# zju3dv/ENeRF

Hardware: AMD Instinct MI355X
Metric: rendered frames/sec @512x640 3-src-view (higher is better)
Workload: dtype f32

## Files before the change

enerf_amd/csrc/render.hip:

```cpp
#include "nerf_layout.h"

#ifndef ENERF_RENDER_PREFETCH
#define ENERF_RENDER_PREFETCH 0
#endif

namespace enerf {

__host__ __device__ __forceinline__ int bx_image_floats(int F, int pieces = 3) { return F == 11 ? bx_layout().tiles * 256 * pieces : 0; }
long long nerf_packed_floats(int F) { return nerf_layout(F).total + bx_image_floats(F); }

__host__ __device__ __forceinline__ int slot_channel(int g, int r, int R, int F) {
    int c = g * R + r;
    return (r < R && c < F) ? c : -1;
}

__device__ __forceinline__ float bx_weight(const NerfRaw& w, int F, int e, int g, int j, int q) {
    const int R = (F + 3) / 4, CI = 88 + F + 4;
    const BxLayout B = bx_layout();
    const int half = q >> 2, r = q & 3;
    const int c = (r < R && g * R + r < F) ? g * R + r : -1;
    if (e < B.ga) return c >= 0 ? w.glob_w[(16 * e + j) * 3 * F + (1 + half) * F + c] : 0.f;
    if (e < B.fc) return (half == 0 && c >= 0) ? w.glob_w[(16 * (e - B.ga) + j) * 3 * F + c] : 0.f;
    if (e < B.lr0) return w.fc_w[j * 32 + 16 * half + 4 * g + r];
    if (e < B.c0p) {
// ... 21 lines not shown
    int i = blockIdx.x * blockDim.x + threadIdx.x;
    if (i >= L.total + bx_image_floats(F)) return;
    if (i >= L.total) {
        const int idx = i - L.total, n_plane = bx_layout().tiles * 256;
        const int piece = idx / n_plane, k = idx - piece * n_plane;
        const int e = k >> 8, lane = (k >> 2) & 63, wq = k & 3;
        unsigned word = 0;
        for (int h = 0; h < 2; ++h) {
            float rem = bx_weight(w, F, e, lane >> 4, lane & 15, 2 * wq + h);
            unsigned bits = 0;
            for (int pc = 0; pc <= piece; ++pc) { bits = bf16_bits_rne(rem); rem -= __uint_as_float(bits << 16); }
            word |= (bits & 0xffffu) << (16 * h);
        }
        out[i] = __uint_as_float(word);
        return;
    }
    const int R = L.R;
    const int CI = 88 + F + 4;
    float v = 0.f;
    auto mfma_lane = [&](int rel, int& e, int& g, int& row) { e = rel >> 6; g = (rel & 63) >> 4; row = rel & 15; };
    int e, g, row;
    if (i >= L.col2) {
        int k = i - L.col2;
        if (k < 64) v = w.col2_w[k]; else if (k == 64) v = w.col2_b[0];
    } else if (i >= L.c0v) {
        mfma_lane(i - L.c0v, e, g, row);
        int ks = e >> 2, vt = e & 3, unit = 16 * vt + row;
        if (ks < R) { int c = slot_channel(g, ks, R, F); if (c >= 0) v = w.col0_w[unit * CI + 88 + c]; }
        else if (ks == R) v = w.col0_w[unit * CI + 88 + F + g];
    } else if (i >= L.c0b) {
        int k = i - L.c0b; if (k < 64) v = w.col0_b[k];
    } else if (i >= L.c0p) {
        mfma_lane(i - L.c0p, e, g, row);
        int ks = e >> 2, vt = e & 3, unit = 16 * vt + row;
        if (ks < 16) v = w.col0_w[unit * CI + 16 * (ks >> 2) + 4 * g + (ks & 3)];
        else if (ks < 18) v = w.col0_w[unit * CI + 64 + 2 * g + (ks - 16)];
        else if (ks < 22) v = w.col0_w[unit * CI + 72 + 4 * g + (ks - 18)];
    } else if (i >= L.sigma) {
        int k = i - L.sigma;
        if (k < 64) v = w.sigma_w[k]; else if (k == 64) v = w.sigma_b[0];
    } else if (i >= L.lr0b) {
        int k = i - L.lr0b; if (k < 64) v = w.lr0_b[k];
    } else if (i >= L.lr0) {
        mfma_lane(i - L.lr0, e, g, row);
        int ks = e >> 2, vt = e & 3, unit = 16 * vt + row;
        if (ks < 2) v = w.lr0_w[unit * 24 + 2 * g + ks];
        else if (ks < 6) v = w.lr0_w[unit * 24 + 8 + 4 * g + (ks - 2)];
    } else if (i >= L.fcb) {
        int k = i - L.fcb; if (k < 16) v = w.fc_b[k];
    } else if (i >= L.fc) {
        mfma_lane(i - L.fc, e, g, row);
        if (e < 8) v = w.fc_w[row * 32 + 16 * (e >> 2) + 4 * g + (e & 3)];
    } else if (i >= L.aggw) {
        int k = i - L.aggw;
        if (k < 32) v = w.aggw_w[k]; else if (k == 32) v = w.aggw_b[0];
    } else if (i >= L.globb) {
        int k = i - L.globb; if (k < 32) v = w.glob_b[k];
    } else if (i >= L.glob) {
        mfma_lane(i - L.glob, e, g, row);
        int u = e & 1, pr = e >> 1, part = pr / R, r = pr - part * R;
        int c = slot_channel(g, r, R, F);
        if (part < 3 && c >= 0) v = w.glob_w[(16 * u + row) * 3 * F + part * F + c];
    } else if (i >= L.viewb) {
        int k = i - L.viewb;
        int t = k >> 4, rr = k & 15;
        int c = slot_channel(rr >> 2, 4 * t + (rr & 3), R, F);
        if (t < L.TR && c >= 0 && viewdir_agg) v = w.view_b[c];
    } else {
        mfma_lane(i - L.view, e, g, row);
        int c = slot_channel(row >> 2, 4 * e + (row & 3), R, F);
        if (e < L.TR && c >= 0 && viewdir_agg) v = w.view_w[c * 4 + g];
    }
    out[i] = v;
}
void launch_nerf_pack(const NerfRaw& raw, int F, int viewdir_agg, float* packed, hipStream_t st) {
    int total = (int)nerf_packed_floats(F);
    ENERF_LAUNCH_SIMPLE(k_nerf_pack, cdiv(total, 256), 256, 0, st, raw, F, viewdir_agg, packed);
}

constexpr int kCamStride = 16;

template <int R> struct Stage { static constexpr int kTex = 4 * R, kStride = 4 * R + 8; };

template <int R, int S, int WAVES, int WPE, bool PFK = false, bool LEANK = false, int BX = 0, bool RAW = false>
__global__ __launch_bounds__(64 * WAVES)
#ifndef ENERF_EMU
__attribute__((amdgpu_waves_per_eu(WPE, WPE)))
#endif
void k_render_rays(RenderArgs a) {
    static_assert(BX == 0 || R == 3, "the bf16 image exists for F = 11 only");
    static_assert(!RAW || (BX == 0 && !PFK), "raw samples come from the exact fp32 kernel, one sample at a time");
    constexpr bool BX3 = BX != 0;
    constexpr int NP = BX == 6 ? 3 : 2;
    constexpr int TR = (R + 3) / 4;
    constexpr int TEX = Stage<R>::kTex, SST = Stage<R>::kStride;
    const NerfLayout LF = nerf_layout(a.F);
    const NerfLayout L = nerf_layout(a.F, BX3);
    constexpr int BXP = 25 * 256;
    constexpr int BXF = BX3 ? BXP * NP : 0;
    ENERF_DYN_SMEM(float, smem);
    float* wl = smem;
    const float* bx = smem + L.total;
    auto bxplane = [&](int q) { return bx + q * BXP; };
    float* cam = smem + L.total + BXF;
    float* tcen = cam + a.B * S * kCamStride;
    float* stage_all = tcen + ((a.B * 4 + 15) & ~15);

    {
        constexpr int MAXW4 = (BX3 ? BXF : (R == 3 ? 10560 : 14528)) / 4;
        constexpr int NWI = (MAXW4 + 64 * WAVES - 1) / (64 * WAVES);
        float4 wq[NWI];
        const int n4 = (BX3 ? BXF : L.total) / 4;
        const float* src = a.packed + (BX3 ? LF.total : 0);
        float* dst = BX3 ? smem + L.total : wl;
#pragma unroll
        for (int it = 0; it < NWI; ++it) {
            const int i = (int)threadIdx.x + it * 64 * WAVES;
            wq[it] = *reinterpret_cast<const float4*>(src + (i < n4 ? i : n4 - 1) * 4);
        }
#pragma unroll
        for (int it = 0; it < NWI; ++it) {
            const int i = (int)threadIdx.x + it * 64 * WAVES;
            if (i < n4) *reinterpret_cast<float4*>(dst + i * 4) = wq[it];
        }
        if (BX3) {
            const int so[9] = {LF.view, LF.viewb, LF.globb, LF.aggw, LF.fcb, LF.lr0b, LF.sigma, LF.c0b, LF.col2};
            const int dd[9] = {L.view, L.viewb, L.globb, L.aggw, L.fcb, L.lr0b, L.sigma, L.c0b, L.col2};
            const int nn[9] = {L.TR * 64, L.TR * 16, 32, 33, 16, 64, 65, 64, 65};
            for (int q = 0; q < 9; ++q)
                for (int i = threadIdx.x; i < nn[q]; i += blockDim.x) wl[dd[q] + i] = a.packed[so[q] + i];
        }
    }
    for (int i = threadIdx.x; i < a.B * (S + 1); i += blockDim.x) {
        int b = i / (S + 1), s = i - b * (S + 1);
        const float* E = (s < S) ? a.src_exts + ((long long)b * S + s) * 16 : a.tar_ext + (long long)b * 16;
        double m[16], inv[16];
        for (int k = 0; k < 16; ++k) m[k] = (double)E[k];
        bool ok = inv4x4(m, inv);
        float c0 = ok ? (float)inv[3] : NAN, c1 = ok ? (float)inv[7] : NAN, c2 = ok ? (float)inv[11] : NAN;
        if (s < S) {
            float* c = cam + ((long long)b * S + s) * kCamStride;
            const float* K = a.src_ixts + ((long long)b * S + s) * 9;
            for (int r = 0; r < 3; ++r) {
                double kr[3];
                for (int q = 0; q < 3; ++q) kr[q] = (double)K[r * 3 + q] * (r < 2 ? (double)a.render_scale : 1.0);
                for (int q = 0; q < 4; ++q) {
                    const double v = kr[0] * m[q] + kr[1] * m[4 + q] + kr[2] * m[8 + q];
                    if (q < 3) c[r * 3 + q] = (float)v; else c[9 + r] = (float)v;
                }
            }
            c[12] = c0; c[13] = c1; c[14] = c2; c[15] = 0.f;
        } else {
            tcen[b * 4 + 0] = c0; tcen[b * 4 + 1] = c1; tcen[b * 4 + 2] = c2; tcen[b * 4 + 3] = 0.f;
        }
    }
    __syncthreads();

    const int lane = threadIdx.x & 63, g = lane >> 4, j = lane & 15;
    const int wave_in_block = threadIdx.x >> 6;
    const long long nrays = a.ray_index != nullptr ? (long long)a.ray_count[0] : (long long)a.B * a.N;
    const long long ntiles = cdivl(nrays, 16);
    const bool scatter = a.ray_index != nullptr && a.scatter_rgb != 0;
    const int Ns = a.n_samples;
    const float* wlane = wl + lane;
#define A_VIEW(e) wlane[L.view + (e) * 64]
#define A_GLOB(e) wlane[L.glob + (e) * 64]
#define A_FC(e) wlane[L.fc + (e) * 64]
#define A_LR0(e) wlane[L.lr0 + (e) * 64]
#define A_C0P(e) wlane[L.c0p + (e) * 64]
#define A_C0V(e) wlane[L.c0v + (e) * 64]
    float* stage = stage_all + wave_in_block * ((PFK ? 2 : 1) * S * 16 * SST);
    const int sv = g < S ? g : S - 1;
    float* my_rec = stage + (sv * 16 + j) * SST;
    const float* rd_rec = stage + j * SST + g * R;
    const float* rd_dir = stage + j * SST + TEX + g;

    const long long nbands = gridDim.x < 8 ? gridDim.x : 8;
    const long long xcd_ = blockIdx.x % nbands, nb8 = ((long long)gridDim.x + nbands - 1 - xcd_) / nbands, bi_ = blockIdx.x / nbands;
    const long long t_hi = ntiles * (xcd_ + 1) / nbands;
#ifndef ENERF_RENDER_BALANCE_R9
#define ENERF_RENDER_BALANCE_R9 1
#endif
    const long long t_lo = ntiles * xcd_ / nbands, per_round = nb8 * WAVES, full = (t_hi - t_lo) / per_round;
    const long long rem = (t_hi - t_lo) - full * per_round, rb = rem / nb8, rx = rem - rb * nb8;
    const long long my_rem = rb + (bi_ < rx ? 1 : 0), my_rem_lo = bi_ * rb + (bi_ < rx ? bi_ : rx);
    constexpr bool kBal = R == 3 || ENERF_RENDER_BALANCE_R9;
    const long long n_it = kBal ? full + (wave_in_block < my_rem ? 1 : 0)
                                : full + (full * per_round + bi_ * WAVES + wave_in_block < t_hi - t_lo ? 1 : 0);
    for (long long it = 0; it < n_it; ++it) {
        const long long tile = (it < full || !kBal) ? t_lo + it * per_round + bi_ * WAVES + wave_in_block
                                                    : t_lo + full * per_round + my_rem_lo + wave_in_block;
        long long ray = tile * 16 + j;
        const bool rok = ray < nrays;
        const long long rc = rok ? ray : nrays - 1;
        const long long rr = a.ray_index != nullptr ? (long long)a.ray_index[rc] : rc;
        const int b = (int)(rr / a.N);
        float ox, oy, oz, dx, dy, dz, ru, rv, rn, rf, vn, vf;
        if (a.rays8 != nullptr) {
            const float* rp = a.rays8 + rr * 8;
            const float4 q0 = *reinterpret_cast<const float4*>(rp), q1 = *reinterpret_cast<const float4*>(rp + 4);
            ox = q0.x; oy = q0.y; oz = q0.z; dx = q0.w; dy = q1.x; dz = q1.y; ru = q1.z; rv = q1.w;
            const long long mo = (long long)b * a.map_h * a.map_w;
            const RayBounds rb = ray_bounds(ru, rv, a.depth_map + mo, a.std_map + mo, a.nf_map + 2 * mo, a.map_h, a.map_w,
                                            a.Hr, a.Wr, a.depth_inv);
            rn = rb.rn; rf = rb.rf; vn = rb.vn; vf = rb.vf;
        } else {
            const float* rp = a.rays12 + rr * 12;
            const float4 q0 = *reinterpret_cast<const float4*>(rp), q1 = *reinterpret_cast<const float4*>(rp + 4),
                         q2 = *reinterpret_cast<const float4*>(rp + 8);
            ox = q0.x; oy = q0.y; oz = q0.z; dx = q0.w; dy = q1.x; dz = q1.y; ru = q1.z; rv = q1.w;
            rn = q2.x; rf = q2.y; vn = q2.z; vf = q2.w;
        }
        const unsigned voff = (unsigned)b * (unsigned)(a.D * a.h * a.w * 8) + 2u * g;
        float wxy[4];
        int oxy[4];
        {
            const float gxv = (ru / (float)(a.Wr - 1)) * 2.f - 1.f, gyv = (rv / (float)(a.Hr - 1)) * 2.f - 1.f;
            float ix = gs_unnorm(gxv, a.w), iy = gs_unnorm(gyv, a.h);
            ix = fabsf(ix) < 1e8f ? ix : -10.f;
            iy = fabsf(iy) < 1e8f ? iy : -10.f;
            const float fx = floorf(ix), fy = floorf(iy);
            const int x0 = (int)fx, y0 = (int)fy;
            float wx[2] = {(fx + 1.f) - ix, ix - fx}, wy[2] = {(fy + 1.f) - iy, iy - fy};
            int xo[2], yo[2];
#pragma unroll
            for (int c = 0; c < 2; ++c) {
                const int xx = x0 + c, yy = y0 + c;
                wx[c] = (unsigned)xx < (unsigned)a.w ? wx[c] : 0.f;
                wy[c] = (unsigned)yy < (unsigned)a.h ? wy[c] : 0.f;
                xo[c] = min(max(xx, 0), a.w - 1);
                yo[c] = mul24(min(max(yy, 0), a.h - 1), a.w);
            }
#pragma unroll
            for (int c = 0; c < 4; ++c) { wxy[c] = wx[c & 1] * wy[c >> 1]; oxy[c] = yo[c >> 1] + xo[c & 1]; }
        }
        const float* cb = cam + ((long long)b * S + sv) * kCamStride;
        f32x4 cm0, cm1, cm2, cm3, tc4;
        if (!LEANK) { cm0 = lds4(cb); cm1 = lds4(cb + 4); cm2 = lds4(cb + 8); cm3 = lds4(cb + 12); tc4 = lds4(tcen + b * 4); }
        const unsigned toff = (unsigned)b * (unsigned)(S * a.Hr * a.Wr * TEX) + (unsigned)sv * (unsigned)(a.Hr * a.Wr * TEX);
        const float rcpW = fast_rcp((float)(a.Wr - 1)), rcpH = fast_rcp((float)(a.Hr - 1));

        float Tacc = 1.f;
        constexpr int NSM = (LEANK && R == 3) ? 2 : 8;
        float wk[NSM];
        float rgbacc[R];
#pragma unroll
        for (int r = 0; r < R; ++r) rgbacc[r] = 0.f;
#pragma unroll
        for (int k = 0; k < NSM; ++k) wk[k] = 0.f;

        struct GatherRegs {
            float2 vt[8];
            f32x4 tq[(R <= 3 ? 1 : 2)][4][(R <= 3 ? R : 3)];
            unsigned tp[4];
            float tw[4], wz[2];
            f32x4 dirc;
        };
        constexpr int QB = R <= 3 ? R : 3, NRND = R / QB, NBUF = NRND > 1 ? 2 : 1;
        static_assert(R % QB == 0, "texel chunk rounds");
        const char* const texb = reinterpret_cast<const char*>(a.tex);
        const char* const volb = reinterpret_cast<const char*>(a.vol);
        auto gather_issue = [&](int k, GatherRegs& G) {
            if (LEANK) { cm0 = lds4(cb); cm1 = lds4(cb + 4); cm2 = lds4(cb + 8); cm3 = lds4(cb + 12); tc4 = lds4(tcen + b * 4); }
            float tk = (Ns == 1) ? 0.5f : linspace01(k, Ns);
            float z = rn + (rf - rn) * tk;
            float zz = a.depth_inv ? fast_rcp(clamp_min(z, 1e-6f)) : z;
            float X = ox + dx * zz, Y = oy + dy * zz, Z = oz + dz * zz;
            float dn = a.depth_inv ? (vn - z) * fast_rcp(clamp_min(vn - vf, 1e-6f))
                                   : (z - vn) * fast_rcp(clamp_min(vf - vn, 1e-6f));
            const float px = X * cm0[0] + Y * cm0[1] + Z * cm0[2] + cm2[1];
            const float py = X * cm0[3] + Y * cm1[0] + Z * cm1[1] + cm2[2];
            const float pz = X * cm1[2] + Y * cm1[3] + Z * cm2[0] + cm2[3];
            const float rz = fast_rcp(clamp_min(pz, 1e-6f));
            const float gx = ((px * rz) * rcpW) * 2.f - 1.f, gy = ((py * rz) * rcpH) * 2.f - 1.f;
            const Taps2 t = gs_taps2<true>(gs_unnorm(gx, a.Wr), gs_unnorm(gy, a.Hr), a.Wr, a.Hr);
            const int r0 = mul24(t.y0, a.Wr), r1 = mul24(t.y1, a.Wr);
            G.tp[0] = (toff + (unsigned)mul24(r0 + t.x0, TEX)) * 4u; G.tp[1] = (toff + (unsigned)mul24(r0 + t.x1, TEX)) * 4u;
            G.tp[2] = (toff + (unsigned)mul24(r1 + t.x0, TEX)) * 4u; G.tp[3] = (toff + (unsigned)mul24(r1 + t.x1, TEX)) * 4u;
            G.tw[0] = t.w00; G.tw[1] = t.w01; G.tw[2] = t.w10; G.tw[3] = t.w11;
            float iz = gs_unnorm(dn * 2.f - 1.f, a.D);
            iz = fabsf(iz) < 1e8f ? iz : -10.f;
            const float fz = floorf(iz);
            const int z0 = (int)fz;
            G.wz[0] = (fz + 1.f) - iz; G.wz[1] = iz - fz;
            int zo[2];
#pragma unroll
            for (int c = 0; c < 2; ++c) {
                const int zc = z0 + c;
                G.wz[c] = (unsigned)zc < (unsigned)a.D ? G.wz[c] : 0.f;
                zo[c] = mul24(min(max(zc, 0), a.D - 1), a.h * a.w);
            }
            __builtin_amdgcn_sched_barrier(0);
            if (RAW && a.vol == nullptr) {
#pragma unroll
                for (int c = 0; c < 8; ++c) G.vt[c] = make_float2(0.f, 0.f);
            } else {
#pragma unroll
                for (int c = 0; c < 8; ++c)
                    G.vt[c] = *reinterpret_cast<const float2*>(volb + ((unsigned)(zo[c >> 2] + oxy[c & 3]) * 8u + voff) * 4u);
            }
#pragma unroll
            for (int rd = 0; rd < NBUF; ++rd)
#pragma unroll
                for (int c = 0; c < 4; ++c)
#pragma unroll
                    for (int q = 0; q < QB; ++q) G.tq[rd][c][q] = lds4(reinterpret_cast<const float*>(texb + G.tp[c]) + 4 * (rd * QB + q));
            __builtin_amdgcn_sched_barrier(0);
            float tx = X - tc4[0], ty = Y - tc4[1], tz = Z - tc4[2];
            float sx = X - cm3[0], sy = Y - cm3[1], sz = Z - cm3[2];
            const float tir = fast_rcp(fast_sqrt(tx * tx + ty * ty + tz * tz) + 1e-6f);
            const float sir = fast_rcp(fast_sqrt(sx * sx + sy * sy + sz * sz) + 1e-6f);
            tx *= tir; ty *= tir; tz *= tir;
            sx *= sir; sy *= sir; sz *= sir;
            const float ex = tx - sx, ey = ty - sy, ez = tz - sz;
            const float eir = fast_rcp(fmaxf(fast_sqrt(ex * ex + ey * ey + ez * ez), 1e-6f));
            G.dirc = f32x4{ex * eir, ey * eir, ez * eir, tx * sx + ty * sy + tz * sz};
        };
        auto gather_finish = [&](GatherRegs& G, float* rec, float (&vox)[2]) {
            float vw[8];
#pragma unroll
            for (int c = 0; c < 8; ++c) vw[c] = wxy[c & 3] * G.wz[c >> 2];
            __builtin_amdgcn_sched_barrier(0);
            f32x4 blend[R];
#pragma unroll
            for (int rd = 0; rd < NRND; ++rd) {
#pragma unroll
                for (int q = 0; q < QB; ++q) {
                    f32x4 acc = G.tq[rd % NBUF][0][q] * G.tw[0];
                    acc += G.tq[rd % NBUF][1][q] * G.tw[1];
                    acc += G.tq[rd % NBUF][2][q] * G.tw[2];
                    acc += G.tq[rd % NBUF][3][q] * G.tw[3];
                    blend[rd * QB + q] = acc;
// ... 105 lines not shown
#pragma unroll
                for (int s = 0; s < S; ++s) {
                    gf[s][0] = relu4(gf[s][0]); gf[s][1] = relu4(gf[s][1]);
                    float part = dot4(gf[s][1], aggw1, dot4(gf[s][0], aggw0, 0.f));
                    aw[s] = relu1(group_sum(part) + aggb);
                }
            } else {
            mfma_chain<2 * R, 2>(P, [&](int e) { return A_GLOB(2 * R + e); },
                                 [&](int ks) { return ks < R ? var[ks < R ? ks : 0] : mean[ks >= R ? ks - R : 0]; });
            {
                float ag[R * 2];
#pragma unroll
                for (int e = 0; e < R * 2; ++e) ag[e] = A_GLOB(e);
                __builtin_amdgcn_sched_barrier(0);
#pragma unroll
                for (int s = 0; s < S; ++s) {
                    gf[s][0] = P[0]; gf[s][1] = P[1];
#pragma unroll
                    for (int r = 0; r < R; ++r)
#pragma unroll
                        for (int u = 0; u < 2; ++u) gf[s][u] = ENERF_MFMA(ag[r * 2 + u], av[s][r], gf[s][u]);
                }
#pragma unroll
                for (int s = 0; s < S; ++s) {
                    gf[s][0] = relu4(gf[s][0]); gf[s][1] = relu4(gf[s][1]);
                    float part = dot4(gf[s][1], aggw1, dot4(gf[s][0], aggw0, 0.f));
                    aw[s] = relu1(group_sum(part) + aggb);
                }
            }
            }
            {
                float m = aw[0];
#pragma unroll
                for (int s = 1; s < S; ++s) m = fmaxf(m, aw[s]);
                float se = 0.f;
#pragma unroll
                for (int s = 0; s < S; ++s) { aw[s] = fast_exp(aw[s] - m); se += aw[s]; }
                se = fast_rcp(se);
#pragma unroll
                for (int s = 0; s < S; ++s) aw[s] *= se;
            }
            f32x4 G[2];
#pragma unroll
            for (int u = 0; u < 2; ++u) {
                G[u] = gf[0][u] * aw[0];
#pragma unroll
                for (int s = 1; s < S; ++s) G[u] += gf[s][u] * aw[s];
            }
            f32x4 aggv[1] = {lds4(wl + L.fcb + 4 * g)};
            if constexpr (BX3) {
                const BxLayout BL = bx_layout();
                bfx8 gp[NP];
                bx_split<NP>(G[0], G[1], gp);
                bx_mma_n<NP, 1>(bxplane, BL.fc, lane, gp, aggv);
            } else {
                float afc[8];
#pragma unroll
                for (int e = 0; e < 8; ++e) afc[e] = A_FC(e);
                __builtin_amdgcn_sched_barrier(0);
#pragma unroll
                for (int e = 0; e < 8; ++e) aggv[0] = ENERF_MFMA(afc[e], G[e >> 2][e & 3], aggv[0]);
            }
            const f32x4 agg = relu4(aggv[0]);

            if (more) gather_finish(GR, my_rec + ((k + 1) & 1) * RECBUF, vox_next);

            f32x4 hid[4];
#pragma unroll
            for (int v = 0; v < 4; ++v) hid[v] = lds4(wl + L.lr0b + v * 16 + 4 * g);
            bfx8 vap[NP];
            if constexpr (BX3) {
                const BxLayout BL = bx_layout();
                bx_split<NP>(f32x4{vox[0], vox[1], 0.f, 0.f}, agg, vap);
                bx_mma_n<NP, 4>(bxplane, BL.lr0, lane, vap, hid);
            } else
            mfma_chain<6, 4>(hid, [&](int e) { return A_LR0(e); }, [&](int ks) { return ks < 2 ? vox[ks < 2 ? ks : 0] : agg[ks >= 2 ? ks - 2 : 0]; });
            float sig = 0.f;
#pragma unroll
            for (int v = 0; v < 4; ++v) {
                hid[v] = relu4(hid[v]);
                sig = dot4(hid[v], lds4(wl + L.sigma + v * 16 + 4 * g), sig);
            }
            sig = group_sum(sig) + wl[L.sigma + 64];
            sig = sig > 20.f ? sig : log1pf(expf(sig));

            f32x4 P2[4];
#pragma unroll
            for (int v = 0; v < 4; ++v) P2[v] = lds4(wl + L.c0b + v * 16 + 4 * g);
            if constexpr (BX3) {
                const BxLayout BL = bx_layout();
#pragma unroll
                for (int pr = 0; pr < 2; ++pr) {
                    bfx8 hp[NP];
                    bx_split<NP>(hid[2 * pr], hid[2 * pr + 1], hp);
                    bx_mma_n<NP, 4>(bxplane, BL.c0p + 4 * pr, lane, hp, P2);
                }
                bx_mma_n<NP, 4>(bxplane, BL.c0p + 8, lane, vap, P2);
            } else
            mfma_chain<22, 4>(P2, [&](int e) { return A_C0P(e); },
                              [&](int ks) { return ks < 16 ? hid[(ks < 16 ? ks : 0) >> 2][ks & 3]
                                                           : (ks < 18 ? vox[ks < 18 ? ks - 16 : 0] : agg[ks >= 18 ? ks - 18 : 0]); });
            float cl[S];
            const float c2b = wl[L.col2 + 64];
            if constexpr (BX3) {
                const BxLayout BL = bx_layout();
                const f32x4 zero4 = {0.f, 0.f, 0.f, 0.f};
                f32x4 c2w[4];
#pragma unroll
                for (int v = 0; v < 4; ++v) c2w[v] = lds4(wl + L.col2 + v * 16 + 4 * g);
#pragma unroll
                for (int s = 0; s < S; ++s) {
                    bfx8 xp[NP];
                    bx_split<NP>(f32x4{x[s][0], x[s][1], x[s][2], dsel[s]}, zero4, xp);
                    f32x4 cc[4] = {P2[0], P2[1], P2[2], P2[3]};
                    bx_mma_n<NP, 4>(bxplane, BL.c0v, lane, xp, cc);
                    float part = 0.f;
#pragma unroll
                    for (int v = 0; v < 4; ++v) part = dot4(relu4(cc[v]), c2w[v], part);
                    cl[s] = relu1(group_sum(part) + c2b);
                }
            } else
            {
                float acv[(R + 1) * 4];
#pragma unroll
                for (int e = 0; e < (R + 1) * 4; ++e) acv[e] = A_C0V(e);
                f32x4 c2w[4];
#pragma unroll
                for (int v = 0; v < 4; ++v) c2w[v] = lds4(wl + L.col2 + v * 16 + 4 * g);
                __builtin_amdgcn_sched_barrier(0);
#pragma unroll
                for (int s = 0; s < S; ++s) {
                    f32x4 cc[4];
#pragma unroll
                    for (int v = 0; v < 4; ++v) cc[v] = P2[v];
#pragma unroll
                    for (int ks = 0; ks <= R; ++ks) {
                        float bop = ks < R ? x[s][ks < R ? ks : 0] : dsel[s];
#pragma unroll
                        for (int v = 0; v < 4; ++v) cc[v] = ENERF_MFMA(acv[ks * 4 + v], bop, cc[v]);
                    }
                    float part = 0.f;
#pragma unroll
                    for (int v = 0; v < 4; ++v) part = dot4(relu4(cc[v]), c2w[v], part);
                    cl[s] = relu1(group_sum(part) + c2b);
                }
            }
            {
                float m = cl[0];
#pragma unroll
                for (int s = 1; s < S; ++s) m = fmaxf(m, cl[s]);
                float se = 0.f;
#pragma unroll
                for (int s = 0; s < S; ++s) { cl[s] = fast_exp(cl[s] - m); se += cl[s]; }
                se = fast_rcp(se);
#pragma unroll
                for (int s = 0; s < S; ++s) cl[s] *= se;
            }

            if constexpr (RAW) {
                const float tk = (Ns == 1) ? 0.5f : linspace01(k, Ns);
                const float zs = rn + (rf - rn) * tk;
                if (rok) {
                    const long long so = ray * Ns + k;
#pragma unroll
                    for (int r = 0; r < R; ++r) {
                        const int c = g * R + r - (a.F - 3);
                        if (c >= 0 && c < 3) {
                            float col = x[0][r] * cl[0];
#pragma unroll
                            for (int s = 1; s < S; ++s) col += x[s][r] * cl[s];
                            a.rgb[so * 4 + c] = col;
                        }
                    }
                    if (g == 0) {
                        a.rgb[so * 4 + 3] = sig;
                        a.depth[so] = a.depth_inv ? 1.f / zs : zs;
                    }
                }
                continue;
            }
            float alpha = 1.f - fast_exp(-sig);
            float wgt = alpha * Tacc;
            Tacc *= (1.f - alpha + 1e-10f);
#pragma unroll
            for (int r = 0; r < R; ++r) {
                float col = x[0][r] * cl[0];
#pragma unroll
                for (int s = 1; s < S; ++s) col += x[s][r] * cl[s];
                rgbacc[r] += wgt * col;
            }
#pragma unroll
            for (int kk = 0; kk < NSM; ++kk)
                if (kk == k) wk[kk] = wgt;
        }
        if constexpr (RAW) continue;

        float m = wk[0];
#pragma unroll
        for (int k = 1; k < NSM; ++k) if (k < Ns) m = fmaxf(m, wk[k]);
        float se = 0.f;
#pragma unroll
        for (int k = 0; k < NSM; ++k) if (k < Ns) { wk[k] = fast_exp(wk[k] - m); se += wk[k]; }
        se = fast_rcp(se);
        float depth = 0.f, accw = 0.f;
#pragma unroll
        for (int k = 0; k < NSM; ++k)
            if (k < Ns) {
                wk[k] *= se;
                float tk = (Ns == 1) ? 0.5f : linspace01(k, Ns);
                depth += wk[k] * (rn + (rf - rn) * tk);
                accw += wk[k];
            }
        if (rok) {
#pragma unroll
            for (int r = 0; r < R; ++r) {
                int c = g * R + r - (a.F - 3);
                if (c >= 0 && c < 3) {
                    float v = rgbacc[r];
                    if (a.white_bkgd) v += 1.f - accw;
                    if (!scatter) a.rgb[ray * 3 + c] = v;
                    else if (nrays > 1) a.rgb[rr * 3 + c] = v;
                }
            }
            if (g == 0) {
                a.depth[ray] = depth;
#pragma unroll
                for (int k = 0; k < NSM; ++k) if (k < Ns) a.weights[ray * Ns + k] = wk[k];
            }
        }
    }
}

template <int R, int WAVES, int OCC, bool PFK = false, bool LEANK = false, int BX3 = 0>
static int dispatch_s(const RenderArgs& a, unsigned grid, size_t shmem, hipStream_t st) {
    constexpr int WPE = (WAVES * OCC + 3) / 4;
    switch (a.S) {
        case 2: ENERF_LAUNCH((k_render_rays<R, 2, WAVES, WPE, PFK, LEANK, BX3>), grid, 64 * WAVES, shmem, st, a); return 0;
        case 3: ENERF_LAUNCH((k_render_rays<R, 3, WAVES, WPE, PFK, LEANK, BX3>), grid, 64 * WAVES, shmem, st, a); return 0;
        case 4: ENERF_LAUNCH((k_render_rays<R, 4, WAVES, WPE, PFK, LEANK, BX3>), grid, 64 * WAVES, shmem, st, a); return 0;
        default: return -3;
    }
}
template <int R, int WAVES, int OCC, bool LEANK>
static int dispatch_s_raw(const RenderArgs& a, unsigned grid, size_t shmem, hipStream_t st) {
    constexpr int WPE = (WAVES * OCC + 3) / 4;
    switch (a.S) {
        case 2: ENERF_LAUNCH((k_render_rays<R, 2, WAVES, WPE, false, LEANK, 0, true>), grid, 64 * WAVES, shmem, st, a); return 0;
        case 3: ENERF_LAUNCH((k_render_rays<R, 3, WAVES, WPE, false, LEANK, 0, true>), grid, 64 * WAVES, shmem, st, a); return 0;
        case 4: ENERF_LAUNCH((k_render_rays<R, 4, WAVES, WPE, false, LEANK, 0, true>), grid, 64 * WAVES, shmem, st, a); return 0;
        default: return -3;
    }
}
template <int R, int WAVES>
static size_t render_shmem(const RenderArgs& a, int record_buffers = 1, int bx = 0) {
    return ((size_t)nerf_layout(a.F, bx != 0).total + (size_t)(bx ? bx_image_floats(a.F, bx == 6 ? 3 : 2) : 0) + (size_t)a.B * a.S * kCamStride + (size_t)((a.B * 4 + 15) & ~15) +
            (size_t)WAVES * record_buffers * a.S * 16 * Stage<R>::kStride) * sizeof(float);
}
int launch_render_rays(const RenderArgs& a, hipStream_t st) {
    if (a.n_samples < 1 || a.n_samples > 8) return -1;
    const int R = (a.F + 3) / 4;
    if ((long long)a.B * a.S * a.Hr * a.Wr * 4 * R >= (1LL << 30) || (long long)a.B * a.D * a.h * a.w * 8 >= (1LL << 30) ||
        (long long)a.Hr * a.Wr >= (1LL << 23) || (long long)a.h * a.w >= (1LL << 23) || a.D >= (1 << 23))
        return -5;
    const long long ntiles = cdivl((long long)a.B * a.N, 16);
    const int cus = device_cu_count();
    auto grid_for = [&](int waves, int occ) {
        const long long blocks = cdivl(ntiles, waves);
        long long resident = (long long)cus * occ;
        if (a.max_blocks > 0 && a.max_blocks < resident) resident = a.max_blocks;
        return (unsigned)(blocks < resident ? blocks : resident);
    };
#ifndef ENERF_R9_LEAN
#define ENERF_R9_LEAN 1
#endif
#ifndef ENERF_RENDER_LEAN12
#define ENERF_RENDER_LEAN12 1
#endif
#ifndef ENERF_RENDER_WAVES
#define ENERF_RENDER_WAVES 4
#endif
#ifndef ENERF_RENDER_OCC
#define ENERF_RENDER_OCC 2
#endif
    if (nerf_layout(a.F).total > (R == 3 ? 10560 : 14528)) return -6;
    if (R == 3 && a.n_samples <= 2 && ENERF_RENDER_LEAN12) {
        const int prec = a.options != nullptr ? a.options->render_precision : 0;
        const int bx = prec == 2 ? 3 : (prec == 3 ? 6 : 0);
        const size_t shmem = render_shmem<3, 12>(a, 1, bx);
        if (shmem <= 160 * 1024) {
            const unsigned grid = grid_for(12, 1);
            if (grid == 0) return 0;
            if (bx == 6) return dispatch_s<3, 12, 1, false, true, 6>(a, grid, shmem, st);
            if (bx == 3) return dispatch_s<3, 12, 1, false, true, 3>(a, grid, shmem, st);
            return dispatch_s<3, 12, 1, false, true>(a, grid, shmem, st);
        }
    }
    if (R == 3) {
        const size_t shmem = render_shmem<3, ENERF_RENDER_WAVES>(a);
        if (shmem > 160 * 1024 / ENERF_RENDER_OCC) return -2;
        const unsigned grid = grid_for(ENERF_RENDER_WAVES, ENERF_RENDER_OCC);
        if (grid == 0) return 0;
        const size_t shmem_pf = render_shmem<3, ENERF_RENDER_WAVES>(a, 2);
        if (ENERF_RENDER_PREFETCH != 0 && a.n_samples > 1 && shmem_pf <= 160 * 1024 / ENERF_RENDER_OCC)
            return dispatch_s<3, ENERF_RENDER_WAVES, ENERF_RENDER_OCC, true>(a, grid, shmem_pf, st);
        return dispatch_s<3, ENERF_RENDER_WAVES, ENERF_RENDER_OCC>(a, grid, shmem, st);
    }
    if (R == 9) {
        const size_t shmem = render_shmem<9, 8>(a);
        if (shmem > 160 * 1024) return -2;
        unsigned grid = grid_for(8, 1);
        if (0 && ENERF_RENDER_BALANCE_R9 && ntiles > 0) {
            const long long t = cdivl(ntiles, 4LL * cus), tight = cdivl(ntiles, 4 * t);
            if (tight < (long long)grid) grid = (unsigned)tight;
        }
        if (grid == 0) return 0;
        return dispatch_s<9, 8, 1, false, ENERF_R9_LEAN != 0>(a, grid, shmem, st);
    }
    return -4;
}

int render_rays_raw_check(const RenderArgs& a) {
    if (a.n_samples < 1 || a.n_samples > 8) return -1;
    const int R = (a.F + 3) / 4;
    if ((long long)a.B * a.S * a.Hr * a.Wr * 4 * R >= (1LL << 30) || (long long)a.B * a.D * a.h * a.w * 8 >= (1LL << 30) ||
        (long long)a.Hr * a.Wr >= (1LL << 23) || (long long)a.h * a.w >= (1LL << 23) || a.D >= (1 << 23))
        return -5;
    if (nerf_layout(a.F).total > (R == 3 ? 10560 : 14528)) return -6;
    if (R != 3 && R != 9) return -4;
    if (R == 3 ? render_shmem<3, ENERF_RENDER_WAVES>(a) > 160 * 1024 / ENERF_RENDER_OCC : render_shmem<9, 8>(a) > 160 * 1024) return -2;
    if (a.S < 2 || a.S > 4) return -3;
    return 0;
}
int launch_render_rays_raw(const RenderArgs& a, hipStream_t st) {
    if (const int rc = render_rays_raw_check(a)) return rc;
    const int R = (a.F + 3) / 4;
    const long long ntiles = cdivl((long long)a.B * a.N, 16);
    const int cus = device_cu_count();
    auto grid_for = [&](int waves, int occ) {
        const long long blocks = cdivl(ntiles, waves);
        long long resident = (long long)cus * occ;
        if (a.max_blocks > 0 && a.max_blocks < resident) resident = a.max_blocks;
        return (unsigned)(blocks < resident ? blocks : resident);
    };
    if (R == 3) {
        const size_t shmem = render_shmem<3, ENERF_RENDER_WAVES>(a);
        if (shmem > 160 * 1024 / ENERF_RENDER_OCC) return -2;
        const unsigned grid = grid_for(ENERF_RENDER_WAVES, ENERF_RENDER_OCC);
        if (grid == 0) return 0;
        return dispatch_s_raw<3, ENERF_RENDER_WAVES, ENERF_RENDER_OCC, false>(a, grid, shmem, st);
    }
    if (R == 9) {
        const size_t shmem = render_shmem<9, 8>(a);
        if (shmem > 160 * 1024) return -2;
        const unsigned grid = grid_for(8, 1);
        if (grid == 0) return 0;
        return dispatch_s_raw<9, 8, 1, ENERF_R9_LEAN != 0>(a, grid, shmem, st);
    }
    return -4;
}

}
```

enerf_amd/lib.py:

```python
from __future__ import annotations

import contextlib
import ctypes as C
import os
import threading
from typing import Optional

import torch

_PKG = os.path.dirname(os.path.abspath(__file__))
LIB_PATH = os.path.join(_PKG, "libenerf_hip.so")
ABI_VERSION = 11

_f = C.c_void_p
_i = C.c_int
_ll = C.c_longlong
_fl = C.c_float


class ConvBn(C.Structure):
    _fields_ = [("w", _f), ("bn_weight", _f), ("bn_bias", _f), ("bn_mean", _f), ("bn_var", _f)]


class CostRegRaw(C.Structure):
    _fields_ = [("conv", ConvBn * 12), ("feat_conv_w", _f), ("depth_conv_w", _f), ("in_channels", _i), ("full", _i)]


class FeatNetRaw(C.Structure):
    _fields_ = [("conv", ConvBn * 6)] + [(n, _f) for n in ("toplayer_w", "toplayer_b", "lat1_w", "lat1_b", "lat0_w",
                                                            "lat0_b", "smooth1_w", "smooth1_b", "smooth0_w", "smooth0_b")]


class NerfRaw(C.Structure):
    _fields_ = [(n, _f) for n in ("view_w", "view_b", "glob_w", "glob_b", "aggw_w", "aggw_b", "fc_w", "fc_b",
                                  "lr0_w", "lr0_b", "sigma_w", "sigma_b", "col0_w", "col0_b", "col2_w", "col2_b")]


class Options(C.Structure):
    _fields_ = [("conv3d_global_only", _i), ("conv3d_lds_min_voxels", _ll), ("conv3d_pk8", _i),
                ("featnet_unfused", _i), ("featnet_smooth0_plain", _i), ("conv3d_b4", _i), ("single_stream", _i),
                ("side_gate", _i), ("fuse_depth_prep", _i), ("conv3d_t2_variant", _i), ("conv3d_small_variant", _i),
                ("render_precision", _i), ("heads_keep_feat", _i)]

    def __repr__(self):
        return "Options(" + ", ".join(f"{n}={getattr(self, n)}" for n, _ in self._fields_ if getattr(self, n)) + ")"


def throughput_options() -> "Options":
    return Options(single_stream=1)


def _opt(o):
    return None if o is None else C.byref(o)


class MlpBwdArgs(C.Structure):
    _fields_ = ([(n, _f) for n in ("vox", "x", "g_raw", "packed", "bimg", "g_vox", "g_x")] + [("save", C.c_void_p * 16),
                ("P", _ll), ("F", _i), ("S", _i), ("image_offsets", _i * 8)])


class GatherArgs(C.Structure):
    _fields_ = ([(n, _f) for n in ("xyz", "dn", "uv", "tex", "vol", "cam", "tcen", "x", "vox", "g_x", "g_vox", "g_tex",
                                   "g_vol", "g_xyz", "g_dn")]
                + [("P", _ll)] + [(n, _i) for n in ("B", "S", "F", "Hr", "Wr", "D", "h", "w", "ray_w", "n_samples")])


class GemmWgradDesc(C.Structure):
    _fields_ = [("a", _f), ("lda", _i), ("Ca", _i), ("b", _f), ("ldb", _i), ("Cb", _i), ("P", _ll), ("grad_w", _f), ("ldw", _i),
                ("grad_bias", _f), ("partials", _f), ("partial_chunks", _i)]


class RenderArgs(C.Structure):
    _fields_ = ([(n, _f) for n in ("rays12", "tex", "vol", "src_exts", "src_ixts", "tar_ext", "packed", "rgb",
                                   "depth", "weights")]
                + [(n, _i) for n in ("B", "N", "S", "n_samples", "depth_inv", "Hr", "Wr", "F", "D", "h", "w",
                                     "white_bkgd")]
                + [("render_scale", _fl)]
                + [(n, _f) for n in ("rays8", "depth_map", "std_map", "nf_map")] + [("map_h", _i), ("map_w", _i)]
                + [("options", C.POINTER(Options)), ("ray_index", C.c_void_p), ("ray_count", C.c_void_p),
                   ("scatter_rgb", _i), ("max_blocks", _i)])


class RenderRawArgs(C.Structure):
    _fields_ = ([(n, _f) for n in ("rays12", "rays8", "depth_map", "std_map", "nf_map")] + [("map_h", _i), ("map_w", _i)]
                + [(n, _f) for n in ("tex", "vol", "src_exts", "src_ixts", "tar_ext", "packed", "raw", "z")]
                + [(n, _i) for n in ("B", "N", "S", "n_samples", "depth_inv", "Hr", "Wr", "F", "D", "h", "w")]
                + [("render_scale", _fl), ("ray_index", C.c_void_p), ("ray_count", C.c_void_p), ("max_blocks", _i)])


MAX_FG_LAYERS = 4


class CompositeLayersArgs(C.Structure):
    _fields_ = ([("fg_raw", C.c_void_p * MAX_FG_LAYERS), ("fg_z", C.c_void_p * MAX_FG_LAYERS), ("win", (_i * 4) * MAX_FG_LAYERS),
                 ("bg_raw", _f), ("bg_z", _f)] + [(n, _i) for n in ("L", "Ns", "H", "W", "white_bkgd")]
                + [(n, _f) for n in ("rgb", "depth", "weights", "net_output", "z_vals")])


class CompositeLayersBwdArgs(C.Structure):
    _fields_ = [("fwd", CompositeLayersArgs), ("grad_rgb", _f), ("grad_depth", _f), ("grad_weights", _f),
                ("grad_fg_raw", C.c_void_p * MAX_FG_LAYERS), ("grad_bg_raw", _f)]


MAX_LEVELS = 3
STAGE_COUNT = 2 + 6 * MAX_LEVELS
STAGE_NAMES = ["begin", "feature_net"] + [f"{n}_{i}" for i in range(MAX_LEVELS)
                                          for n in ("prep", "volume", "cost_reg", "depth_reg", "texels", "render")]
_dL, _iL, _fL = C.c_double * MAX_LEVELS, C.c_int * MAX_LEVELS, C.c_void_p * MAX_LEVELS


class Cascade(C.Structure):
    _fields_ = [("num", _i), ("depth_inv", _iL), ("volume_scale", _dL), ("volume_planes", _iL), ("im_feat_scale", _dL),
                ("im_ibr_scale", _dL), ("render_scale", _dL), ("render_im_feat_level", _iL), ("nerf_model_feat_ch", _iL),
                ("render_if", _iL), ("num_samples", _iL), ("white_bkgd", _i)]


class FrameArgs(C.Structure):
    _fields_ = ([(n, _f) for n in ("src_inps", "src_exts", "src_ixts", "tar_ext", "tar_ixt", "near_far")]
                + [("rays", _fL), ("n_rays", _iL), ("mask_at_box", C.c_void_p), ("mask_elem_bytes", _i)]
                + [(n, _i) for n in ("B", "S", "H", "W")] + [("cas", Cascade)]
                + [("feature_net_packed", _f), ("cost_reg_packed", _fL), ("nerf_packed", _fL), ("feats_nchw", C.c_void_p * 3)]
                + [(n, _fL) for n in ("rgb", "depth", "weights", "depth_mvs", "std")]
                + [("ray_index", C.c_void_p), ("ray_count", C.c_void_p), ("ray_index_ready", _i),
                   ("workspace", C.c_void_p), ("workspace_bytes", C.c_size_t), ("options", C.POINTER(Options)),
                   ("stage_events", C.POINTER(C.c_void_p))])
# ... 1671 lines not shown
```

include/enerf_hip.h:

```cpp
#ifndef ENERF_HIP_H_
#define ENERF_HIP_H_

#include <stddef.h>

#ifdef __cplusplus
extern "C" {
#endif

#define ENERF_ABI_VERSION 11
#define ENERF_OK 0
#define ENERF_EINVAL (-1)
#define ENERF_ELAUNCH (-2)
#define ENERF_EWORKSPACE (-3)

typedef void* enerf_stream_t;

int enerf_abi_version(void);
const char* enerf_last_error(void);

int enerf_selftest_checks(void);
int enerf_selftest_primitives(const float* table, int table_floats, float* scratch, int blocks, unsigned* mismatches, enerf_stream_t stream);

typedef struct {
    int conv3d_global_only;
    long long conv3d_lds_min_voxels;
    int conv3d_pk8;
    int featnet_unfused;
    int featnet_smooth0_plain;
    int conv3d_b4;
    int single_stream;
    int side_gate;
    int fuse_depth_prep;
    int conv3d_t2_variant;
    int conv3d_small_variant;
    int render_precision;
    int heads_keep_feat;
} enerf_options_t;

int enerf_channels_last(const float* src, float* dst, int n, int C, long long P, int Cpad, enerf_stream_t stream);
int enerf_channels_first(const float* src, float* dst, int n, int C, long long P, int Cpad, enerf_stream_t stream);

int enerf_pack_img_feat_rgb(const float* im_feat, int C, int Hf, int Wf, const float* src_inps, int H, int W,
                            int Hr, int Wr, int tex, int n_img, float* out, enerf_stream_t stream);

typedef struct {
    const float* w;
    const float* bn_weight;
    const float* bn_bias;
    const float* bn_mean;
    const float* bn_var;
} enerf_conv_bn_t;

typedef struct {
    enerf_conv_bn_t conv[6];
    const float *toplayer_w, *toplayer_b;
    const float *lat1_w, *lat1_b;
    const float *lat0_w, *lat0_b;
    const float *smooth1_w, *smooth1_b;
    const float *smooth0_w, *smooth0_b;
} enerf_featnet_raw_t;
long long enerf_feature_net_packed_floats(void);
int enerf_feature_net_pack(const enerf_featnet_raw_t* raw, float* packed, enerf_stream_t stream);
size_t enerf_feature_net_workspace_bytes(int n_img, int H, int W);
int enerf_feature_net(const float* packed, const float* src_inps, int n_img, int H, int W, float* feat_l0,
                      float* feat_l1, float* feat_l2, int l2_stride, void* workspace, size_t workspace_bytes,
                      const enerf_options_t* options, enerf_stream_t stream);
enum { ENERF_FEAT_ALL = 0, ENERF_FEAT_TRUNK = 1, ENERF_FEAT_LEVEL1 = 2, ENERF_FEAT_LEVEL2 = 3 };
int enerf_feature_net_stage(const float* packed, const float* src_inps, int n_img, int H, int W, float* feat_l0,
                            float* feat_l1, float* feat_l2, int l2_stride, void* workspace, size_t workspace_bytes,
                            int stage, const enerf_options_t* options, enerf_stream_t stream);
int enerf_pack_texels_cl(const float* feat_cl, int C, const float* src_inps, int H, int W, int Hr, int Wr, int tex,
                         int n_img, float* out, enerf_stream_t stream);

int enerf_get_proj_mats(const float* src_ixts, const float* src_exts, const float* tar_ixt, const float* tar_ext,
                        int B, int S, float src_scale, float tar_scale, float* proj, enerf_stream_t stream);

int enerf_get_depth_values(const float* near_far, const float* prev_depth, const float* prev_std,
                           const float* prev_near_far, int B, int D, int h, int w, int hp, int wp, int depth_inv,
                           float* depth_values, float* near_far_out, enerf_stream_t stream);
int enerf_level_prep(const float* src_ixts, const float* src_exts, const float* tar_ixt, const float* tar_ext, int B,
                     int S, float src_scale, float tar_scale, float* proj, const float* near_far,
                     const float* prev_depth, const float* prev_std, const float* prev_near_far, int D, int h, int w,
                     int hp, int wp, int depth_inv, float* depth_values, float* near_far_out, enerf_stream_t stream);

int enerf_build_feature_volume(const float* feat, const float* proj, const float* depth_values, int B, int S, int C,
                               int Hs, int Ws, int D, int h, int w, float* vol, enerf_stream_t stream);

typedef struct {
    enerf_conv_bn_t conv[12];
    const float* feat_conv_w;
    const float* depth_conv_w;
    int in_channels;
    int full;
} enerf_costreg_raw_t;
long long enerf_cost_reg_packed_floats(int in_channels, int full);
int enerf_cost_reg_pack(const enerf_costreg_raw_t* raw, float* packed, enerf_stream_t stream);
size_t enerf_cost_reg_workspace_bytes(int full, int B, int D, int h, int w);
int enerf_cost_reg(const float* packed, int in_channels, int full, const float* vol, int B, int D, int h, int w,
                   float* feat, float* prob, void* workspace, size_t workspace_bytes, const enerf_options_t* options,
                   enerf_stream_t stream);
int enerf_cost_reg_prob(const float* packed, int in_channels, int full, const float* vol, int B, int D, int h, int w, float* prob,
                        void* workspace, size_t workspace_bytes, const enerf_options_t* options, enerf_stream_t stream);

int enerf_depth_regression(const float* prob, const float* depth_values, int B, int D, int h, int w, int depth_inv,
                           float* depth, float* std, enerf_stream_t stream);

int enerf_build_rays(const float* rays8, const float* depth, const float* std, const float* near_far, int B, int N,
                     int h, int w, int Hr, int Wr, int depth_inv, float* rays12, enerf_stream_t stream);

typedef struct {
    const float *view_w, *view_b;
    const float *glob_w, *glob_b;
    const float *aggw_w, *aggw_b;
    const float *fc_w, *fc_b;
    const float *lr0_w, *lr0_b;
    const float *sigma_w, *sigma_b;
    const float *col0_w, *col0_b;
    const float *col2_w, *col2_b;
} enerf_nerf_raw_t;
// ... 421 lines not shown
```

Measured before the change: 1338.

## Share per-ray setup across tiles and batch softplus/compositing per lane in lean renderer

```diff
diff --git a/enerf_amd/csrc/render.hip b/enerf_amd/csrc/render.hip
--- a/enerf_amd/csrc/render.hip
+++ b/enerf_amd/csrc/render.hip
@@ -127,7 +127,8 @@
 
 template <int R> struct Stage { static constexpr int kTex = 4 * R, kStride = 4 * R + 8; };
 
-template <int R, int S, int WAVES, int WPE, bool PFK = false, bool LEANK = false, int BX = 0, bool RAW = false>
+constexpr int kShareStride = 20;
+template <int R, int S, int WAVES, int WPE, bool PFK = false, bool LEANK = false, int BX = 0, bool RAW = false, int TS = 0>
 __global__ __launch_bounds__(64 * WAVES)
 #ifndef ENERF_EMU
 __attribute__((amdgpu_waves_per_eu(WPE, WPE)))
@@ -135,6 +136,7 @@
 void k_render_rays(RenderArgs a) {
     static_assert(BX == 0 || R == 3, "the bf16 image exists for F = 11 only");
     static_assert(!RAW || (BX == 0 && !PFK), "raw samples come from the exact fp32 kernel, one sample at a time");
+    static_assert(TS == 0 || ((TS == 2 || TS == 4) && R == 3 && LEANK && BX == 0 && !RAW && !PFK), "tile sharing: the lean level-1 build only");
     constexpr bool BX3 = BX != 0;
     constexpr int NP = BX == 6 ? 3 : 2;
     constexpr int TR = (R + 3) / 4;
@@ -150,6 +152,7 @@
     float* cam = smem + L.total + BXF;
     float* tcen = cam + a.B * S * kCamStride;
     float* stage_all = tcen + ((a.B * 4 + 15) & ~15);
+    float* share_all = stage_all + WAVES * ((PFK ? 2 : 1) * S * 16 * SST);
 
     {
         constexpr int MAXW4 = (BX3 ? BXF : (R == 3 ? 10560 : 14528)) / 4;
@@ -232,15 +235,28 @@
     constexpr bool kBal = R == 3 || ENERF_RENDER_BALANCE_R9;
     const long long n_it = kBal ? full + (wave_in_block < my_rem ? 1 : 0)
                                 : full + (full * per_round + bi_ * WAVES + wave_in_block < t_hi - t_lo ? 1 : 0);
+    constexpr int GT = TS != 0 ? TS : 1;
+    float* const share = share_all + wave_in_block * (GT * 16 * kShareStride);
     for (long long it = 0; it < n_it; ++it) {
         const long long tile = (it < full || !kBal) ? t_lo + it * per_round + bi_ * WAVES + wave_in_block
                                                     : t_lo + full * per_round + my_rem_lo + wave_in_block;
         long long ray = tile * 16 + j;
         const bool rok = ray < nrays;
-        const long long rc = rok ? ray : nrays - 1;
-        const long long rr = a.ray_index != nullptr ? (long long)a.ray_index[rc] : rc;
-        const int b = (int)(rr / a.N);
+        long long rr;
+        int b;
         float ox, oy, oz, dx, dy, dz, ru, rv, rn, rf, vn, vf;
+        float wxy[4];
+        int oxy[4];
+        if (TS == 0 || (it & (GT - 1)) == 0) {
+        long long ray_s = ray;
+        if constexpr (TS != 0) {
+            const long long left = n_it - it, its = it + (g < left ? g : left - 1);
+            ray_s = ((its < full || !kBal) ? t_lo + its * per_round + bi_ * WAVES + wave_in_block
+                                           : t_lo + full * per_round + my_rem_lo + wave_in_block) * 16 + j;
+        }
+        const long long rc = (TS != 0 ? ray_s < nrays : rok) ? ray_s : nrays - 1;
+        rr = a.ray_index != nullptr ? (long long)a.ray_index[rc] : rc;
+        b = (int)(rr / a.N);
         if (a.rays8 != nullptr) {
             const float* rp = a.rays8 + rr * 8;
             const float4 q0 = *reinterpret_cast<const float4*>(rp), q1 = *reinterpret_cast<const float4*>(rp + 4);
@@ -256,9 +272,6 @@
             ox = q0.x; oy = q0.y; oz = q0.z; dx = q0.w; dy = q1.x; dz = q1.y; ru = q1.z; rv = q1.w;
             rn = q2.x; rf = q2.y; vn = q2.z; vf = q2.w;
         }
-        const unsigned voff = (unsigned)b * (unsigned)(a.D * a.h * a.w * 8) + 2u * g;
-        float wxy[4];
-        int oxy[4];
         {
             const float gxv = (ru / (float)(a.Wr - 1)) * 2.f - 1.f, gyv = (rv / (float)(a.Hr - 1)) * 2.f - 1.f;
             float ix = gs_unnorm(gxv, a.w), iy = gs_unnorm(gyv, a.h);
@@ -279,6 +292,28 @@
 #pragma unroll
             for (int c = 0; c < 4; ++c) { wxy[c] = wx[c & 1] * wy[c >> 1]; oxy[c] = yo[c >> 1] + xo[c & 1]; }
         }
+        if constexpr (TS != 0) {
+            if (g < GT) {
+                float* sp = share + (g * 16 + j) * kShareStride;
+                *reinterpret_cast<f32x4*>(sp) = f32x4{ox, oy, oz, dx};
+                *reinterpret_cast<f32x4*>(sp + 4) = f32x4{dy, dz, rn, rf};
+                *reinterpret_cast<f32x4*>(sp + 8) = f32x4{vn, vf, __int_as_float(b), __int_as_float((int)rr)};
+                *reinterpret_cast<f32x4*>(sp + 12) = f32x4{wxy[0], wxy[1], wxy[2], wxy[3]};
+                *reinterpret_cast<f32x4*>(sp + 16) = f32x4{__int_as_float(oxy[0]), __int_as_float(oxy[1]), __int_as_float(oxy[2]), __int_as_float(oxy[3])};
+            }
+            wave_sync();
+        }
+        }
+        if constexpr (TS != 0) {
+            const float* sp = share + (((int)it & (GT - 1)) * 16 + j) * kShareStride;
+            const f32x4 s0 = lds4(sp), s1 = lds4(sp + 4), s2 = lds4(sp + 8), s3 = lds4(sp + 12), s4 = lds4(sp + 16);
+            ox = s0[0]; oy = s0[1]; oz = s0[2]; dx = s0[3]; dy = s1[0]; dz = s1[1]; rn = s1[2]; rf = s1[3];
+            vn = s2[0]; vf = s2[1]; b = __float_as_int(s2[2]);
+            rr = (long long)__float_as_int(s2[3]);
+#pragma unroll
+            for (int c = 0; c < 4; ++c) { wxy[c] = s3[c]; oxy[c] = __float_as_int(s4[c]); }
+        }
+        const unsigned voff = (unsigned)b * (unsigned)(a.D * a.h * a.w * 8) + 2u * g;
         const float* cb = cam + ((long long)b * S + sv) * kCamStride;
         f32x4 cm0, cm1, cm2, cm3, tc4;
         if (!LEANK) { cm0 = lds4(cb); cm1 = lds4(cb + 4); cm2 = lds4(cb + 8); cm3 = lds4(cb + 12); tc4 = lds4(tcen + b * 4); }
@@ -293,6 +328,14 @@
         for (int r = 0; r < R; ++r) rgbacc[r] = 0.f;
 #pragma unroll
         for (int k = 0; k < NSM; ++k) wk[k] = 0.f;
+        constexpr int NSK = TS != 0 ? NSM : 1;
+        float sigk[NSK], colk[NSK][R];
+#pragma unroll
+        for (int k = 0; k < NSK; ++k) {
+            sigk[k] = 0.f;
+#pragma unroll
+            for (int r = 0; r < R; ++r) colk[k][r] = 0.f;
+        }
 
         struct GatherRegs {
             float2 vt[8];
@@ -564,7 +607,7 @@
                 sig = dot4(hid[v], lds4(wl + L.sigma + v * 16 + 4 * g), sig);
             }
             sig = group_sum(sig) + wl[L.sigma + 64];
-            sig = sig > 20.f ? sig : log1pf(expf(sig));
+            if constexpr (TS == 0) sig = sig > 20.f ? sig : log1pf(expf(sig));
 
             f32x4 P2[4];
 #pragma unroll
@@ -661,6 +704,21 @@
                 }
                 continue;
             }
+            if constexpr (TS != 0) {
+#pragma unroll
+                for (int kk = 0; kk < NSM; ++kk)
+                    if (kk == k) sigk[kk] = sig;
+#pragma unroll
+                for (int r = 0; r < R; ++r) {
+                    float col = x[0][r] * cl[0];
+#pragma unroll
+                    for (int s = 1; s < S; ++s) col += x[s][r] * cl[s];
+#pragma unroll
+                    for (int kk = 0; kk < NSM; ++kk)
+                        if (kk == k) colk[kk][r] = col;
+                }
+                continue;
+            }
             float alpha = 1.f - fast_exp(-sig);
             float wgt = alpha * Tacc;
             Tacc *= (1.f - alpha + 1e-10f);
@@ -676,6 +734,27 @@
                 if (kk == k) wk[kk] = wgt;
         }
         if constexpr (RAW) continue;
+        if constexpr (TS != 0) {
+            float sg = sigk[0];
+#pragma unroll
+            for (int k = 1; k < NSK; ++k) sg = g == k ? sigk[k] : sg;
+            sg = sg > 20.f ? sg : log1pf(expf(sg));
+            if (g < Ns) stage[g * 16 + j] = sg;
+            wave_sync();
+#pragma unroll
+            for (int k = 0; k < NSK; ++k) sigk[k] = k < Ns ? stage[k * 16 + j] : 0.f;
+            wave_sync();
+#pragma unroll
+            for (int k = 0; k < NSK; ++k)
+                if (k < Ns) {
+                    float alpha = 1.f - fast_exp(-sigk[k]);
+                    float wgt = alpha * Tacc;
+                    Tacc *= (1.f - alpha + 1e-10f);
+#pragma unroll
+                    for (int r = 0; r < R; ++r) rgbacc[r] += wgt * colk[k][r];
+                    wk[k] = wgt;
+                }
+        }
 
         float m = wk[0];
 #pragma unroll
@@ -720,6 +799,15 @@
         case 2: ENERF_LAUNCH((k_render_rays<R, 2, WAVES, WPE, PFK, LEANK, BX3>), grid, 64 * WAVES, shmem, st, a); return 0;
         case 3: ENERF_LAUNCH((k_render_rays<R, 3, WAVES, WPE, PFK, LEANK, BX3>), grid, 64 * WAVES, shmem, st, a); return 0;
         case 4: ENERF_LAUNCH((k_render_rays<R, 4, WAVES, WPE, PFK, LEANK, BX3>), grid, 64 * WAVES, shmem, st, a); return 0;
+        default: return -3;
+    }
+}
+constexpr int render_share_tiles(int S) { return S <= 3 ? 4 : 2; }
+static int dispatch_s_share(const RenderArgs& a, unsigned grid, size_t shmem, hipStream_t st) {
+    switch (a.S) {
+        case 2: ENERF_LAUNCH((k_render_rays<3, 2, 12, 3, false, true, 0, false, render_share_tiles(2)>), grid, 64 * 12, shmem, st, a); return 0;
+        case 3: ENERF_LAUNCH((k_render_rays<3, 3, 12, 3, false, true, 0, false, render_share_tiles(3)>), grid, 64 * 12, shmem, st, a); return 0;
+        case 4: ENERF_LAUNCH((k_render_rays<3, 4, 12, 3, false, true, 0, false, render_share_tiles(4)>), grid, 64 * 12, shmem, st, a); return 0;
         default: return -3;
     }
 }
@@ -774,6 +862,9 @@
             if (grid == 0) return 0;
             if (bx == 6) return dispatch_s<3, 12, 1, false, true, 6>(a, grid, shmem, st);
             if (bx == 3) return dispatch_s<3, 12, 1, false, true, 3>(a, grid, shmem, st);
+            const bool share = !(a.options != nullptr && a.options->render_tile_share == 1) && a.S >= 2 && a.S <= 4;
+            const size_t shmem_ts = shmem + (size_t)12 * render_share_tiles(a.S) * 16 * kShareStride * sizeof(float);
+            if (share && shmem_ts <= 160 * 1024) return dispatch_s_share(a, grid, shmem_ts, st);
             return dispatch_s<3, 12, 1, false, true>(a, grid, shmem, st);
         }
     }
diff --git a/enerf_amd/lib.py b/enerf_amd/lib.py
--- a/enerf_amd/lib.py
+++ b/enerf_amd/lib.py
@@ -40,7 +40,7 @@
     _fields_ = [("conv3d_global_only", _i), ("conv3d_lds_min_voxels", _ll), ("conv3d_pk8", _i),
                 ("featnet_unfused", _i), ("featnet_smooth0_plain", _i), ("conv3d_b4", _i), ("single_stream", _i),
                 ("side_gate", _i), ("fuse_depth_prep", _i), ("conv3d_t2_variant", _i), ("conv3d_small_variant", _i),
-                ("render_precision", _i), ("heads_keep_feat", _i)]
+                ("render_precision", _i), ("heads_keep_feat", _i), ("render_tile_share", _i)]
 
     def __repr__(self):
         return "Options(" + ", ".join(f"{n}={getattr(self, n)}" for n, _ in self._fields_ if getattr(self, n)) + ")"
diff --git a/include/enerf_hip.h b/include/enerf_hip.h
--- a/include/enerf_hip.h
+++ b/include/enerf_hip.h
@@ -35,6 +35,7 @@
     int conv3d_small_variant;
     int render_precision;
     int heads_keep_feat;
+    int render_tile_share;
 } enerf_options_t;
 
 int enerf_channels_last(const float* src, float* dst, int n, int C, long long P, int Cpad, enerf_stream_t stream);
```

Result: no change. 1347, median of 6 (+0.7%).
